# osmarks/meme-search-engine

Hardware: AMD Instinct MI355X
Metric: queries/sec over 1e8x1152 index @ recall@10>=0.95 (exact brute force: recall 1.0) (higher is better)
Workload: dtype f16 in, f32 accumulate, i64 fixed-point scores; 1 GPU; brute-force top-10 over 100000000 x 1152 fp16 rows, 320 queries/step, row-sharded over 1 GPU(s); rows_total=100000000, rows_per_gpu=100000000, k=10, parallelism=row-shard x1

## Files before the change

### meme-search-engine_amd/csrc/scan_mfma.hip

```cpp
#include "common.h"
#include "kernels.h"
#include <cstdlib>
#include <algorithm>
#include <type_traits>

namespace mse {
namespace {

typedef _Float16 half8 __attribute__((ext_vector_type(8)));
typedef float float4v __attribute__((ext_vector_type(4)));
typedef uint32_t u32x4 __attribute__((ext_vector_type(4)));

constexpr int KB = 64;
constexpr int W = 8;
constexpr int TILE_ROWS = 32 * W;

__global__ void pack_queries_kernel(const uint16_t* __restrict__ queries, int d, int bn, int n_rows, uint4* __restrict__ packed) {
    const int nkb = d / KB;
    const int QT_SLOTS = bn * 8;
    const int total = nkb * QT_SLOTS;
    queries += (size_t)blockIdx.y * bn * d;
    n_rows -= blockIdx.y * bn;
    packed += (size_t)blockIdx.y * total;
    for (int idx = blockIdx.x * blockDim.x + threadIdx.x; idx < total; idx += gridDim.x * blockDim.x) {
        const int kb = idx / QT_SLOTS;
        const int r = idx % QT_SLOTS;
        const int q = r >> 3, slot_sw = r & 7;
        const int slot = slot_sw ^ ((q >> 1) & 7);
        packed[idx] = q < n_rows ? *reinterpret_cast<const uint4*>(queries + (size_t)q * d + kb * KB + slot * 8) : uint4{0u, 0u, 0u, 0u};
    }
}

__device__ __forceinline__ half8 as_half8(const u32x4& v) { return __builtin_bit_cast(half8, v); }

template <int N> __device__ __forceinline__ void vm_wait() {
    asm volatile("s_waitcnt vmcnt(%0)" ::"n"(N) : "memory");
    __builtin_amdgcn_sched_barrier(0);
}
__device__ __forceinline__ void dma16(const void* gptr, void* lds_wave_base) {
    __builtin_amdgcn_global_load_lds((const __attribute__((address_space(1))) void*)gptr,
                                     (__attribute__((address_space(3))) void*)lds_wave_base, 16, 0, 0);
}

constexpr float MASKED_OUT = -3.402823466e+38f;
__device__ __forceinline__ uint32_t group_word(size_t group, const uint32_t* words, size_t n_words) {
    return group < n_words ? words[group] : 0u;
}

template <int S, int NCT, int ABL = 0, typename... Mask>
__global__ __launch_bounds__(W * 64) void scan_mfma_kernel(const uint16_t* __restrict__ base, size_t n_rows, int d,
                                                           const uint4* __restrict__ packed_ro,
                                                           float* __restrict__ gmax, int nq_pad, size_t n_tiles, uint32_t y_packed, uint32_t y_cols,
                                                           Mask... mask) {
    constexpr int BN = NCT * 16;
    constexpr int QT_BYTES = BN * 128;
    constexpr int QI = BN / 64;
    constexpr bool ILV = S >= 2 && !(ABL & 16);
    extern __shared__ __attribute__((aligned(16))) char smem[];
    const int tid = threadIdx.x;
    const int lane = tid & 63, wave = tid >> 6;
    const int i = lane & 15, g = lane >> 4;
    const int nkb = d / KB;
    const size_t row_bytes = (size_t)d * 2;
    const int swz = (i >> 1) & 7;
    const size_t n_groups = (n_rows + 31) / 32;
    char* const qbase = smem;
    char* const xbase = smem + 2 * QT_BYTES + wave * (S * 4096);
    gmax += (size_t)blockIdx.y * y_cols;
    const char* const packed = reinterpret_cast<const char*>(packed_ro + (size_t)blockIdx.y * y_packed) + (size_t)(wave * QI * 64 + lane) * 16;

    size_t tile = blockIdx.x;
    if (tile >= n_tiles) return;

    auto src_ptr = [&](size_t t, int u) -> const char* {
        const int r = 8 * u + (lane >> 3);
        size_t row = t * TILE_ROWS + wave * 32 + r;
        if (row >= n_rows) row = n_rows - 1;
        const int piece = (lane & 7) ^ ((r >> 1) & 7);
        return reinterpret_cast<const char*>(base) + row * row_bytes + piece * 16;
    };
    auto dma_x = [&](const char* (&rp)[4], int kblock, int stage) {
        char* dst = xbase + stage * 4096;
        if (ABL & 4) return;
#pragma unroll
        for (int u = 0; u < 4; u++) dma16(rp[u] + (size_t)kblock * 128, dst + u * 1024);
    };
    auto dma_q = [&](int kblock, int qb) {
        const char* src = packed + (size_t)kblock * QT_BYTES;
        char* dst = qbase + qb * QT_BYTES + wave * (QI * 1024);
        if (ABL & 2) return;
#pragma unroll
        for (int u = 0; u < QI; u++) dma16(src + u * 1024, dst + u * 1024);
    };

    const char* rp[4];
    const char* rn[4];
#pragma unroll
    for (int u = 0; u < 4; u++) rp[u] = src_ptr(tile, u);
    dma_q(0, 0);
#pragma unroll
    for (int j = 0; j < S - 1; j++) dma_x(rp, j % nkb, j);
    vm_wait<0>();
    __builtin_amdgcn_s_barrier();

    int buf = 0;
    while (true) {
        float4v acc[2][NCT];
#pragma unroll
        for (int rt = 0; rt < 2; rt++)
#pragma unroll
            for (int ct = 0; ct < NCT; ct++)
#pragma unroll
                for (int r = 0; r < 4; r++) acc[rt][ct][r] = 0.0f;

        const size_t next_tile = tile + gridDim.x;
        const bool has_next_tile = next_tile < n_tiles;
#pragma unroll
        for (int u = 0; u < 4; u++) rn[u] = has_next_tile ? src_ptr(next_tile, u) : rp[u];

        for (int kb0 = 0; kb0 < nkb; kb0 += S) {
#pragma unroll
            for (int j = 0; j < S; j++) {
                const int kb = kb0 + j;
                const int kq = kb + 1 == nkb ? 0 : kb + 1;
                const int kf = kb + S - 1;
                const bool x_next = kf >= nkb;
                const size_t xoff = (size_t)(kf >= nkb ? kf - nkb : kf) * 128;
                char* const xdst = xbase + ((j + S - 1) % S) * 4096;
                const char* const qsrc = packed + (size_t)kq * QT_BYTES;
                char* const qdst = qbase + (buf ^ 1) * QT_BYTES + wave * (QI * 1024);
                auto issue_piece = [&](int p) {
                    if (p < QI) { if (!(ABL & 2)) dma16(qsrc + p * 1024, qdst + p * 1024); }
                    else if (!(ABL & 4)) dma16((x_next ? rn[p - QI] : rp[p - QI]) + xoff, xdst + (p - QI) * 1024);
                };
                if (!ILV) {
#pragma unroll
                    for (int p = 0; p < QI + 4; p++) issue_piece(p);
                    vm_wait<(QI + 4) * (S - 1)>();
                } else if (S == 2) {
                    vm_wait<0>();
                }

                const u32x4* xs = reinterpret_cast<const u32x4*>(xbase + j * 4096) + i * 8;
                const u32x4* qt = reinterpret_cast<const u32x4*>(qbase + buf * QT_BYTES) + i * 8;
                const int slot_a = g ^ swz, slot_b = (4 + g) ^ swz;
                u32x4 bq[2][2];
                bq[0][0] = qt[0 * 128 + slot_a];
                bq[0][1] = qt[1 * 128 + slot_a];
                const half8 a00 = as_half8(xs[slot_a]), a10 = as_half8(xs[128 + slot_a]);
                const half8 a01 = as_half8(xs[slot_b]), a11 = as_half8(xs[128 + slot_b]);
                constexpr int NCP = NCT / 2;
#pragma unroll
                for (int t = 0; t < 2 * NCP; t++) {
                    const int ks = t / NCP, cp = t % NCP;
                    if (t + 1 < 2 * NCP) {
                        const int ks2 = (t + 1) / NCP, cp2 = (t + 1) % NCP;
                        if (!(ABL & 8)) {
                            bq[(t + 1) & 1][0] = qt[(cp2 * 2) * 128 + (ks2 ? slot_b : slot_a)];
                            bq[(t + 1) & 1][1] = qt[(cp2 * 2 + 1) * 128 + (ks2 ? slot_b : slot_a)];
                        } else {
                            bq[(t + 1) & 1][0] = bq[t & 1][1];
                            bq[(t + 1) & 1][1] = bq[t & 1][0];
                        }
                    }
                    __builtin_amdgcn_sched_barrier(0);
                    if (ILV) {
                        constexpr int STEP = (2 * NCP) / (QI + 4);
                        if (t >= 1 && (t - 1) % STEP == 0 && (t - 1) / STEP < QI + 4) {
                            issue_piece((t - 1) / STEP);
                            __builtin_amdgcn_sched_barrier(0);
                        }
                    }
                    const half8 a0 = ks ? a01 : a00;
                    const half8 a1 = ks ? a11 : a10;
#pragma unroll
                    for (int e = 0; e < 2; e++) {
                        const half8 b = as_half8(bq[t & 1][e]);
                        const int ct = cp * 2 + e;
                        if (!(ABL & 1)) {
                            acc[0][ct] = __builtin_amdgcn_mfma_f32_16x16x32_f16(a0, b, acc[0][ct], 0, 0, 0);
                            acc[1][ct] = __builtin_amdgcn_mfma_f32_16x16x32_f16(a1, b, acc[1][ct], 0, 0, 0);
                        } else {
                            asm volatile("" ::"v"(b), "v"(a0), "v"(a1));
                        }
                    }
                }
                vm_wait<4>();
                __builtin_amdgcn_s_barrier();
                buf ^= 1;
            }
        }

        const size_t group = tile * W + wave;
        if constexpr (sizeof...(Mask) != 0) {
            const uint32_t w = group_word(group, mask...) >> (4 * g);
#pragma unroll
            for (int rt = 0; rt < 2; rt++)
#pragma unroll
                for (int r = 0; r < 4; r++) {
                    if ((w >> (16 * rt + r)) & 1u) continue;
#pragma unroll
                    for (int ct = 0; ct < NCT; ct++) acc[rt][ct][r] = MASKED_OUT;
                }
        }
#pragma unroll
        for (int ct = 0; ct < NCT; ct++) {
            float m = fmaxf(fmaxf(acc[0][ct][0], acc[0][ct][1]), fmaxf(acc[0][ct][2], acc[0][ct][3]));
            m = fmaxf(m, fmaxf(fmaxf(acc[1][ct][0], acc[1][ct][1]), fmaxf(acc[1][ct][2], acc[1][ct][3])));
            m = fmaxf(m, __shfl_xor(m, 16));
            m = fmaxf(m, __shfl_xor(m, 32));
            if (g == 0 && group < n_groups) gmax[group * (size_t)nq_pad + ct * 16 + i] = m;
        }

        if (!has_next_tile) break;
        tile = next_tile;
#pragma unroll
        for (int u = 0; u < 4; u++) rp[u] = rn[u];
    }
    vm_wait<0>();
}


typedef float float16v __attribute__((ext_vector_type(16)));

#ifdef MSE_DEV_KERNELS
__device__ unsigned long long g_scan_prof[4];
__device__ __forceinline__ uint32_t memtime() { return (uint32_t)__builtin_amdgcn_s_memtime(); }
#endif

template <typename... M> struct is_tile_subset : std::false_type {};
template <> struct is_tile_subset<ScanSparse> : std::true_type {};
template <typename... M> __device__ __forceinline__ ScanSparse tile_subset_of(const M&...) { return ScanSparse{}; }
__device__ __forceinline__ ScanSparse tile_subset_of(const ScanSparse& sp) { return sp; }

template <int S, int MF, int PROF = 0, int BN = 256, int GR = 32, typename... Mask>
__global__ __launch_bounds__(W * 64) void scan_mfma2d_kernel(const uint16_t* __restrict__ base, size_t n_rows, int d,
                                                             const uint4* __restrict__ packed_ro,
                                                             float* __restrict__ gmax, int nq_pad, size_t n_tiles, uint32_t y_packed, uint32_t y_cols,
                                                             Mask... mask) {
    constexpr bool SPF = is_tile_subset<Mask...>::value;
    constexpr bool MASKED = sizeof...(Mask) != 0 && !SPF;
    static_assert(sizeof...(Mask) == 0 || (MF == 16 && PROF == 0), "the masked form is the product kernel's");
    static_assert(!SPF || (BN == 320 && GR == 64), "a tile subset: the 320-query search pass only");
    static_assert(BN == 256 || (BN == 320 && MF == 16 && S == 2), "320 queries: 16x16x32 tiles on the two-stage ring only");
    static_assert(GR == 32 || (GR == 64 && MF == 16), "rows per written maximum: 32, or the wave's 64");
    constexpr int HALF = BN / 2;
    constexpr int QT_BYTES = BN * 128;
    constexpr int QI = BN / 64;
    constexpr bool XF = S == 2 && PROF != 4;
    constexpr int CLOSE = S == 2 ? 0 : 4;
    constexpr int RG_BYTES = 64 * 128;
    extern __shared__ __attribute__((aligned(16))) char smem[];
    const int tid = threadIdx.x;
    const int lane = tid & 63, wave = is_tile_subset<Mask...>::value ? __builtin_amdgcn_readfirstlane(tid >> 6) : tid >> 6;
    const int rg = wave >> 1, qh = wave & 1;
    const int nkb = d / KB;
    const size_t row_bytes = (size_t)d * 2;
    const size_t n_groups = (n_rows + GR - 1) / GR;
    char* const qbase = smem;
    char* const xbase = smem + 2 * QT_BYTES + rg * (S * RG_BYTES);
    gmax += (size_t)blockIdx.y * y_cols;
    const char* const packed = reinterpret_cast<const char*>(packed_ro + (size_t)blockIdx.y * y_packed) + (size_t)(wave * QI * 64 + lane) * 16;

    const ScanSparse sp = tile_subset_of(mask...);
    const size_t n_vt = SPF ? sp.n_tiles : n_tiles;
    auto tile_of = [&](size_t v) -> size_t { return SPF ? v * sp.mul + (v >> sp.shift) + sp.add : v; };
    size_t vt = blockIdx.x;
    if (vt >= n_vt) return;
    size_t tile = tile_of(vt);

    auto src_ptr = [&](size_t t, int u) -> const char* {
        const int r = qh * 32 + 8 * u + (lane >> 3);
        size_t row = t * TILE_ROWS + rg * 64 + r;
        if (row >= n_rows) row = n_rows - 1;
        const int piece = (lane & 7) ^ ((r >> 1) & 7);
        return reinterpret_cast<const char*>(base) + row * row_bytes + piece * 16;
    };
    const char* rp[4];
    const char* rn[4];
#pragma unroll
    for (int u = 0; u < 4; u++) rp[u] = src_ptr(tile, u);
    {
        char* qdst = qbase + wave * (QI * 1024);
#pragma unroll
        for (int u = 0; u < QI; u++) dma16(packed + u * 1024, qdst + u * 1024);
#pragma unroll
        for (int j = 0; j < S - 1; j++)
#pragma unroll
            for (int u = 0; u < 4; u++) dma16(rp[u] + (size_t)(j % nkb) * 128, xbase + j * RG_BYTES + (qh * 4 + u) * 1024);
    }
    vm_wait<0>();
    __builtin_amdgcn_s_barrier();

    const int i = MF == 16 ? (lane & 15) : (lane & 31);
    const int g = MF == 16 ? (lane >> 4) : (lane >> 5);
    const int swz = (i >> 1) & 7;
    constexpr int NKS = MF == 16 ? 2 : 4;
    constexpr int NRT = 64 / MF, NCTW = HALF / MF;
    constexpr int NACC = MF == 16 ? 4 : 16;
    typedef typename std::conditional<MF == 16, float4v, float16v>::type accv;

    int buf = 0;
#ifdef MSE_DEV_KERNELS
    uint32_t pt_issue = 0, pt_wait = 0, pt_bar = 0, pt_n = 0, pt_last = 0;
    if constexpr (PROF == 1) pt_last = memtime();
#endif
    while (true) {
        accv acc[NRT][NCTW];
#pragma unroll
        for (int rt = 0; rt < NRT; rt++)
#pragma unroll
            for (int ct = 0; ct < NCTW; ct++)
#pragma unroll
                for (int r = 0; r < NACC; r++) acc[rt][ct][r] = 0.0f;

        const size_t next_vt = vt + gridDim.x;
        const size_t next_tile = tile_of(next_vt);
        const bool has_next_tile = next_vt < n_vt;
#pragma unroll
        for (int u = 0; u < 4; u++) rn[u] = has_next_tile ? src_ptr(next_tile, u) : rp[u];

        for (int kb0 = 0; kb0 < nkb; kb0 += S) {
#pragma unroll
            for (int j = 0; j < S; j++) {
                const int kb = kb0 + j;
                const int kq = kb + 1 == nkb ? 0 : kb + 1;
                const int kf = kb + S - 1;
                const bool x_next = kf >= nkb;
                const size_t xoff = (size_t)(kf >= nkb ? kf - nkb : kf) * 128;
                char* const xdst = xbase + ((j + S - 1) % S) * RG_BYTES + qh * 4096;
                const char* const qsrc = packed + (size_t)kq * QT_BYTES;
                char* const qdst = qbase + (buf ^ 1) * QT_BYTES + wave * (QI * 1024);
                auto issue_piece = [&](int p) {
                    const int pq = XF ? p - 4 : p, px = XF ? p : p - QI;
                    if (XF ? p >= 4 : p < QI) dma16(qsrc + pq * 1024, qdst + pq * 1024);
                    else dma16((x_next ? rn[px] : rp[px]) + xoff, xdst + px * 1024);
                };

                const u32x4* xs = reinterpret_cast<const u32x4*>(xbase + j * RG_BYTES) + i * 8;
                const u32x4* qt = reinterpret_cast<const u32x4*>(qbase + buf * QT_BYTES) + (qh * HALF + i) * 8;
                auto slot = [&](int ks) { return (MF == 16 ? (4 * ks + g) : (2 * ks + g)) ^ swz; };
                half8 a[2][NRT];
#pragma unroll
                for (int rt = 0; rt < NRT; rt++) a[0][rt] = as_half8(xs[rt * (MF * 8) + slot(0)]);
                constexpr int NT = NKS * NCTW;
                u32x4 bq[3];
                bq[0] = qt[0 * (MF * 8) + slot(0)];
                bq[1] = qt[1 * (MF * 8) + slot(0)];
#pragma unroll
                for (int t = 0; t < NT; t++) {
                    const int ks = t / NCTW, ct = t % NCTW;
                    if (t + 2 < NT) bq[(t + 2) % 3] = qt[((t + 2) % NCTW) * (MF * 8) + slot((t + 2) / NCTW)];
                    if (ct == NCTW - 2 && ks + 1 < NKS) {
#pragma unroll
                        for (int rt = 0; rt < NRT; rt++) a[(ks + 1) & 1][rt] = as_half8(xs[rt * (MF * 8) + slot(ks + 1)]);
                    }
                    __builtin_amdgcn_sched_barrier(0);
                    {
                        constexpr int STEP = NT / (QI + 4);
                        int pc = -1;
                        if constexpr (S == 2 && PROF != 4 && PROF != 5 && !MASKED) {
                            if (t >= 1 && t <= 4) pc = t - 1;
                            else if (t >= 6 && (t - 6) % 2 == 0 && (t - 6) / 2 < QI) pc = 4 + (t - 6) / 2;
                        } else if (t >= 1 && (t - 1) % STEP == 0 && (t - 1) / STEP < QI + 4) pc = (t - 1) / STEP;
                        if (pc >= 0) {
                            issue_piece(pc);
                            __builtin_amdgcn_sched_barrier(0);
                        }
                    }
                    const half8 b = as_half8(bq[t % 3]);
                    if constexpr (PROF == 3) __builtin_amdgcn_s_setprio(1);
#pragma unroll
                    for (int rt = 0; rt < NRT; rt++) {
                        if constexpr (MF == 16) acc[rt][ct] = __builtin_amdgcn_mfma_f32_16x16x32_f16(a[ks & 1][rt], b, acc[rt][ct], 0, 0, 0);
                        else acc[rt][ct] = __builtin_amdgcn_mfma_f32_32x32x16_f16(a[ks & 1][rt], b, acc[rt][ct], 0, 0, 0);
                    }
                    if constexpr (PROF == 3) __builtin_amdgcn_s_setprio(0);
                }
#ifdef MSE_DEV_KERNELS
                if constexpr (PROF == 1) {
                    const uint32_t t0 = memtime();
                    vm_wait<CLOSE>();
                    const uint32_t t1 = memtime();
                    __builtin_amdgcn_s_barrier();
                    const uint32_t t2 = memtime();
                    pt_issue += t0 - pt_last; pt_wait += t1 - t0; pt_bar += t2 - t1; pt_n++; pt_last = t2;
                } else
#endif
                {
                    vm_wait<CLOSE>();
#ifdef MSE_DEV_KERNELS
                    if constexpr (PROF != 2)
#endif
                    __builtin_amdgcn_s_barrier();
                }
                buf ^= 1;
            }
        }

        if constexpr (MASKED && GR == 32) {
#pragma unroll
            for (int p = 0; p < 2; p++) {
                const uint32_t w = group_word(tile * W + rg * 2 + p, mask...) >> (4 * g);
#pragma unroll
                for (int h = 0; h < 2; h++)
#pragma unroll
                    for (int r = 0; r < 4; r++) {
                        if ((w >> (16 * h + r)) & 1u) continue;
#pragma unroll
                        for (int ct = 0; ct < NCTW; ct++) acc[2 * p + h][ct][r] = MASKED_OUT;
                    }
            }
        }
        if constexpr (GR == 64) {
            const size_t group = tile * 4 + rg;
            uint32_t allowed = 0xFFFFu;
            if constexpr (MASKED) {
                const uint32_t w0 = group_word(group * 2, mask...) >> (4 * g), w1 = group_word(group * 2 + 1, mask...) >> (4 * g);
                allowed = (w0 & 15u) | ((w0 >> 16 & 15u) << 4) | ((w1 & 15u) << 8) | ((w1 >> 16 & 15u) << 12);
            }
            auto av = [&](int rt, int ct, int r) {
                if constexpr (MASKED) return (allowed >> (4 * rt + r)) & 1u ? acc[rt][ct][r] : MASKED_OUT;
                else return acc[rt][ct][r];
            };
            float tq[3] = {0.0f, 0.0f, 0.0f};
            uint32_t cbase = (uint32_t)(qh * HALF + i);
            if constexpr (SPF) {
                asm volatile("" : "+v"(cbase));
                if (sp.tau) {
#pragma unroll
                    for (int j = 0; j < 3; j++) tq[j] = g + 4 * j < NCTW ? sp.tau[cbase + (g + 4 * j) * MF] : __builtin_inff();
                }
            }
#pragma unroll
            for (int ct = 0; ct < NCTW; ct++) {
                float m = fmaxf(fmaxf(av(0, ct, 0), av(0, ct, 1)), fmaxf(av(0, ct, 2), av(0, ct, 3)));
#pragma unroll
                for (int rt = 1; rt < 4; rt++)
                    m = fmaxf(m, fmaxf(fmaxf(av(rt, ct, 0), av(rt, ct, 1)), fmaxf(av(rt, ct, 2), av(rt, ct, 3))));
                m = fmaxf(m, __shfl_xor(m, 16));
                m = fmaxf(m, __shfl_xor(m, 32));
#ifdef MSE_DEV_KERNELS
                if constexpr (PROF == 6) { asm volatile("" ::"v"(m)); continue; }
#endif
                if constexpr (SPF) {
                    if (sp.tau) {
                        const uint32_t col = cbase + ct * MF;
                        if (g == (ct & 3) && group < n_groups && m > tq[ct >> 2]) {
                            uint32_t one;
                            asm volatile("v_mov_b32 %0, 1" : "=v"(one));
                            const uint32_t pos = atomicAdd(&sp.counts[col], one);
                            if (pos < sp.cap) {
                                sp.ids[col * sp.cap + pos] = (uint32_t)group;
                                sp.keys[col * sp.cap + pos] = m;
                            }
                        }
                    } else if (g == 0 && group < n_groups) {
                        gmax[(vt * 4 + rg) * (size_t)nq_pad + cbase + ct * MF] = m;
                    }
                    __builtin_amdgcn_sched_barrier(0);
                    continue;
                }
                if (g == 0 && group < n_groups) gmax[group * (size_t)nq_pad + qh * HALF + ct * MF + i] = m;
            }
        } else {
#pragma unroll
            for (int p = 0; p < 2; p++) {
                const size_t group = tile * W + rg * 2 + p;
#pragma unroll
                for (int ct = 0; ct < NCTW; ct++) {
                    float m;
                    if constexpr (MF == 16) {
                        m = fmaxf(fmaxf(acc[2 * p][ct][0], acc[2 * p][ct][1]), fmaxf(acc[2 * p][ct][2], acc[2 * p][ct][3]));
                        m = fmaxf(m, fmaxf(fmaxf(acc[2 * p + 1][ct][0], acc[2 * p + 1][ct][1]), fmaxf(acc[2 * p + 1][ct][2], acc[2 * p + 1][ct][3])));
                        m = fmaxf(m, __shfl_xor(m, 16));
                        m = fmaxf(m, __shfl_xor(m, 32));
                    } else {
                        m = acc[p][ct][0];
#pragma unroll
                        for (int r = 1; r < 16; r++) m = fmaxf(m, acc[p][ct][r]);
                        m = fmaxf(m, __shfl_xor(m, 32));
                    }
                    if (g == 0 && group < n_groups) gmax[group * (size_t)nq_pad + qh * HALF + ct * MF + i] = m;
                }
            }
        }

        if (!has_next_tile) break;
        vt = next_vt;
        tile = next_tile;
#pragma unroll
        for (int u = 0; u < 4; u++) rp[u] = rn[u];
#ifdef MSE_DEV_KERNELS
        if constexpr (PROF == 1) pt_last = memtime();
#endif
    }
    vm_wait<0>();
#ifdef MSE_DEV_KERNELS
    if constexpr (PROF == 1) {
        if (lane == 0) {
            atomicAdd(&g_scan_prof[0], (unsigned long long)pt_issue); atomicAdd(&g_scan_prof[1], (unsigned long long)pt_wait);
            atomicAdd(&g_scan_prof[2], (unsigned long long)pt_bar); atomicAdd(&g_scan_prof[3], (unsigned long long)pt_n);
        }
    }
#endif
}


#ifdef MSE_DEV_KERNELS

template <int S>
__global__ __launch_bounds__(W * 64) void scan_mfma2s_kernel(const uint16_t* __restrict__ base, size_t n_rows, int d,
                                                             const uint4* __restrict__ packed_ro,
                                                             float* __restrict__ gmax, int nq_pad, size_t n_tiles, uint32_t y_packed, uint32_t y_cols) {
    static_assert(S == 3, "the specialised schedule is written for the 3-stage ring");
    constexpr int BN = 256;
    constexpr int QT_BYTES = BN * 128;
    constexpr int RG_BYTES = 64 * 128;
    constexpr int NP = 8;
    extern __shared__ __attribute__((aligned(16))) char smem[];
    const int tid = threadIdx.x;
    const int lane = tid & 63;
    const int wave = __builtin_amdgcn_readfirstlane(tid >> 6);
    const int rg = wave >> 1, qh = wave & 1;
    const bool row_wave = wave < 4;
    const int w4 = wave & 3;
    const int nkb = d / KB;
    const size_t row_bytes = (size_t)d * 2;
    char* const qbase = smem;
    char* const xring = smem + 2 * QT_BYTES;
    char* const xbase = xring + rg * (S * RG_BYTES);
    char* const xfill = xring + w4 * (S * RG_BYTES);
    char* const qfill = qbase + w4 * (NP * 1024);
    gmax += (size_t)blockIdx.y * y_cols;
    const char* const packed = reinterpret_cast<const char*>(packed_ro + (size_t)blockIdx.y * y_packed) + (size_t)w4 * (NP * 1024) + lane * 16;

    size_t tile = blockIdx.x;
    if (tile >= n_tiles) return;

    const size_t lane_off = (size_t)(lane >> 3) * row_bytes + (size_t)(((lane & 7) ^ (lane >> 4)) * 16);
    const char* const rows0 = reinterpret_cast<const char*>(base) + (size_t)w4 * 64 * row_bytes;
    auto tile_ptr = [&](size_t t) { return rows0 + t * TILE_ROWS * row_bytes + lane_off; };
    const char* lp = tile_ptr(tile);
    const char* ln = lp;
    const size_t piece_rows = 8 * row_bytes;
    auto dma_row_piece = [&](const char* p, int u, size_t koff, char* dst) {
        const char* q = (u & 1) ? reinterpret_cast<const char*>(reinterpret_cast<uintptr_t>(p) ^ 64u) : p;
        dma16(q + (u * piece_rows + koff), dst + u * 1024);
    };
    if (row_wave) {
#pragma unroll
        for (int j = 0; j < S - 1; j++)
#pragma unroll
            for (int u = 0; u < NP; u++) dma_row_piece(lp, u, (size_t)(j % nkb) * 128, xfill + j * RG_BYTES);
    } else {
#pragma unroll
        for (int u = 0; u < NP; u++) dma16(packed + u * 1024, qfill + u * 1024);
    }
    vm_wait<0>();
    __builtin_amdgcn_s_barrier();

    const int i = lane & 15, g = lane >> 4;
    const int swz = (i >> 1) & 7;
    int buf = 0;
    while (true) {
        float4v acc[4][8];
#pragma unroll
        for (int rt = 0; rt < 4; rt++)
#pragma unroll
            for (int ct = 0; ct < 8; ct++)
#pragma unroll
                for (int r = 0; r < 4; r++) acc[rt][ct][r] = 0.0f;

        const size_t next_tile = tile + gridDim.x;
        const bool has_next_tile = next_tile < n_tiles;
        ln = has_next_tile ? tile_ptr(next_tile) : lp;

        for (int kb0 = 0; kb0 < nkb; kb0 += S) {
#pragma unroll
            for (int j = 0; j < S; j++) {
                const int kb = kb0 + j;
                const int kq = kb + 1 == nkb ? 0 : kb + 1;
                const int kf = kb + S - 1;
                const char* const xp = kf >= nkb ? ln : lp;
                const size_t xoff = (size_t)(kf >= nkb ? kf - nkb : kf) * 128;
                char* const xdst = xfill + ((j + S - 1) % S) * RG_BYTES;
                const char* const qsrc = packed + (size_t)kq * QT_BYTES;
                char* const qdst = qfill + (buf ^ 1) * QT_BYTES;
                auto issue_piece = [&](int p) {
                    if (row_wave) dma_row_piece(xp, p, xoff, xdst);
                    else dma16(qsrc + p * 1024, qdst + p * 1024);
                };

                const u32x4* xs = reinterpret_cast<const u32x4*>(xbase + j * RG_BYTES) + i * 8;
                const u32x4* qt = reinterpret_cast<const u32x4*>(qbase + buf * QT_BYTES) + (qh * 128 + i) * 8;
                auto slot = [&](int ks) { return (4 * ks + g) ^ swz; };
                half8 a[2][4];
#pragma unroll
                for (int rt = 0; rt < 4; rt++) a[0][rt] = as_half8(xs[rt * 128 + slot(0)]);
                u32x4 bq[3];
                bq[0] = qt[0 * 128 + slot(0)];
                bq[1] = qt[1 * 128 + slot(0)];
#pragma unroll
                for (int t = 0; t < 16; t++) {
                    const int ks = t / 8, ct = t % 8;
                    if (t + 2 < 16) bq[(t + 2) % 3] = qt[((t + 2) % 8) * 128 + slot((t + 2) / 8)];
                    if (ct == 6 && ks == 0) {
#pragma unroll
                        for (int rt = 0; rt < 4; rt++) a[1][rt] = as_half8(xs[rt * 128 + slot(1)]);
                    }
                    __builtin_amdgcn_sched_barrier(0);
                    if (t >= 1 && (t - 1) % 2 == 0 && (t - 1) / 2 < NP) {
                        issue_piece((t - 1) / 2);
                        __builtin_amdgcn_sched_barrier(0);
                    }
                    const half8 b = as_half8(bq[t % 3]);
#pragma unroll
                    for (int rt = 0; rt < 4; rt++) acc[rt][ct] = __builtin_amdgcn_mfma_f32_16x16x32_f16(a[ks][rt], b, acc[rt][ct], 0, 0, 0);
                }
                if (row_wave) vm_wait<NP>(); else vm_wait<0>();
                __builtin_amdgcn_s_barrier();
                buf ^= 1;
            }
        }

#pragma unroll
        for (int p = 0; p < 2; p++) {
            const size_t group = tile * W + rg * 2 + p;
#pragma unroll
            for (int ct = 0; ct < 8; ct++) {
                float m = fmaxf(fmaxf(acc[2 * p][ct][0], acc[2 * p][ct][1]), fmaxf(acc[2 * p][ct][2], acc[2 * p][ct][3]));
                m = fmaxf(m, fmaxf(fmaxf(acc[2 * p + 1][ct][0], acc[2 * p + 1][ct][1]), fmaxf(acc[2 * p + 1][ct][2], acc[2 * p + 1][ct][3])));
                m = fmaxf(m, __shfl_xor(m, 16));
                m = fmaxf(m, __shfl_xor(m, 32));
                if (g == 0) gmax[group * (size_t)nq_pad + qh * 128 + ct * 16 + i] = m;
            }
        }
        if (!has_next_tile) break;
        tile = next_tile;
        lp = ln;
    }
    vm_wait<0>();
}
#endif

thread_local unsigned g_pass_count = 1;
thread_local uint32_t g_pass_packed = 0, g_pass_cols = 0;

template <typename K, typename... Mask>
int launch_kernel(K kernel, size_t lds, size_t grid, hipStream_t stream, const uint16_t* base, size_t n_rows, int d,
                  const uint4* packed, float* group_max, int nq_pad, Mask... mask) {
    const size_t n_tiles = (n_rows + TILE_ROWS - 1) / TILE_ROWS;
    if (grid > n_tiles) grid = n_tiles;
    MSE_DYN_LDS(kernel, lds);
    hipLaunchKernelGGL(kernel, dim3((unsigned)grid, g_pass_count), dim3(W * 64), lds, stream, base, n_rows, d, packed, group_max, nq_pad, n_tiles,
                       g_pass_packed, g_pass_cols, mask...);
    MSE_HIP_TRY(hipGetLastError());
    return 0;
}

template <int S, int NCT, int ABL, typename... Mask>
int launch_variant(size_t grid, hipStream_t stream, const uint16_t* base, size_t n_rows, int d, const uint4* packed,
                   float* group_max, int nq_pad, Mask... mask) {
    const size_t lds = 2 * (size_t)(NCT * 16 * 128) + (size_t)W * S * 4096;
    return launch_kernel(scan_mfma_kernel<S, NCT, ABL, Mask...>, lds, grid, stream, base, n_rows, d, packed, group_max, nq_pad, mask...);
}

#ifdef MSE_DEV_KERNELS

template <int S>
int launch_2s(size_t grid, hipStream_t stream, const uint16_t* base, size_t n_rows, int d, const uint4* packed,
              float* group_max, int nq_pad) {
    const size_t lds = 2 * (size_t)(256 * 128) + (size_t)4 * S * 8192;
    const size_t n_full = n_rows / TILE_ROWS * TILE_ROWS;
    if (n_full && launch_kernel(scan_mfma2s_kernel<S>, lds, grid, stream, base, n_full, d, packed, group_max, nq_pad)) return -1;
    if (n_full < n_rows)
        return launch_variant<S, 16, 0>(1, stream, base + n_full * (size_t)d, n_rows - n_full, d, packed,
                                        group_max + (n_full / 32) * (size_t)nq_pad, nq_pad);
    return 0;
}
#endif

template <int S, int MF, int PROF = 0, int BN = 256, int GR = 32, typename... Mask>
int launch_2d(size_t grid, hipStream_t stream, const uint16_t* base, size_t n_rows, int d, const uint4* packed,
              float* group_max, int nq_pad, Mask... mask) {
    const size_t lds = 2 * (size_t)(BN * 128) + (size_t)4 * S * 8192;
    return launch_kernel(scan_mfma2d_kernel<S, MF, PROF, BN, GR, Mask...>, lds, grid, stream, base, n_rows, d, packed, group_max, nq_pad, mask...);
}

}

int mfma_query_tile(int d) { return (d / KB) % 2 == 0 ? 320 : 256; }
int mfma_pad(int nq, int d) {
    if (nq <= 128) return 128;
    if (nq <= 192 && (d / KB) % 3 == 0) return 192;
    if (nq <= 256 || (d / KB) % 2 != 0) return 256;
    return 320;
}

size_t mfma_packed_bytes(int d) { return (size_t)(d / KB) * 320 * 128; }

#ifndef MSE_GROUP_ROWS_320
#define MSE_GROUP_ROWS_320 64
#endif
int mfma_group_rows(int nq_pad) {
#ifdef MSE_DEV_KERNELS
    if (getenv("MSE_SCAN_2D") || (getenv("MSE_SCAN_ABL") && atoi(getenv("MSE_SCAN_ABL")) != 32)) return 32;
#endif
    return nq_pad == 320 ? MSE_GROUP_ROWS_320 : 32;
}

int launch_scan_mfma(const uint16_t* base, size_t n_rows, int d, const uint16_t* queries_dev, int nq_pad,
                     void* packed_scratch, float* group_max, int n_cu, hipStream_t stream, hipEvent_t ev_begin,
                     hipEvent_t ev_end, int gm_stride, int n_pass, const uint32_t* mask, size_t mask_words, int nq_rows, int group_rows) {
    if (n_rows == 0) return 0;
    if (group_rows != 32 && !(group_rows == 64 && nq_pad == 320)) return fail("scan_mfma: 32 rows per group maximum, or 64 on the 320-query pass");
    if (nq_rows < 0) nq_rows = n_pass * nq_pad;
    if (n_pass < 1 || n_pass > 65535) return fail("scan_mfma: 1..65535 passes per launch");
    if (n_pass > 1 && !gm_stride) return fail("scan_mfma: batched passes need a common group-maximum stride");
    const int gs = gm_stride ? gm_stride : nq_pad;
    if (gs < nq_pad) return fail("scan_mfma: group-maximum stride below the pass width");
    if (d % 64 != 0 || d <= 0 || d > D_MAX) return fail("vector width must be a positive multiple of 64");
    if (nq_pad != 128 && nq_pad != 256 && !(nq_pad == 192 && (d / KB) % 3 == 0) && !(nq_pad == 320 && (d / KB) % 2 == 0))
        return fail("scan_mfma: query tile must be padded to 128, 192 (K blocks divisible by 3), 256 or 320 (K blocks even)");
    uint4* packed = reinterpret_cast<uint4*>(packed_scratch);
    hipLaunchKernelGGL(pack_queries_kernel, dim3(64, (unsigned)n_pass), dim3(256), 0, stream, queries_dev, d, nq_pad, nq_rows, packed);
    struct PassScope {
        PassScope(unsigned n, uint32_t pk, uint32_t cols) { g_pass_count = n; g_pass_packed = pk; g_pass_cols = cols; }
        ~PassScope() { g_pass_count = 1; g_pass_packed = 0; g_pass_cols = 0; }
    } pass_scope((unsigned)n_pass, (uint32_t)((size_t)(d / KB) * nq_pad * 8), (uint32_t)nq_pad);
    if (ev_begin) MSE_HIP_TRY(hipEventRecord(ev_begin, stream));
    const int nkb = d / KB;
    const int S = nkb % 3 == 0 ? 3 : nkb % 2 == 0 ? 2 : 1;
    const size_t grid = (size_t)n_cu;
    int rc = -2;
#ifdef MSE_DEV_KERNELS
    if (!mask && group_rows == 32) {
    const int abl = getenv("MSE_SCAN_ABL") ? atoi(getenv("MSE_SCAN_ABL")) : 0;
    const int v2d = getenv("MSE_SCAN_2D") ? atoi(getenv("MSE_SCAN_2D")) : -1;
    if (nq_pad == 128 && S == 3 && abl == 16) rc = launch_variant<3, 8, 16>(grid, stream, base, n_rows, d, packed, group_max, gs);
    else if (nq_pad == 256 && S == 3 && abl) {
        switch (abl) {
            case 1: rc = launch_variant<3, 16, 1>(grid, stream, base, n_rows, d, packed, group_max, gs); break;
            case 2: rc = launch_variant<3, 16, 2>(grid, stream, base, n_rows, d, packed, group_max, gs); break;
            case 4: rc = launch_variant<3, 16, 4>(grid, stream, base, n_rows, d, packed, group_max, gs); break;
            case 6: rc = launch_variant<3, 16, 6>(grid, stream, base, n_rows, d, packed, group_max, gs); break;
            case 8: rc = launch_variant<3, 16, 8>(grid, stream, base, n_rows, d, packed, group_max, gs); break;
            case 9: rc = launch_variant<3, 16, 9>(grid, stream, base, n_rows, d, packed, group_max, gs); break;
            case 14: rc = launch_variant<3, 16, 14>(grid, stream, base, n_rows, d, packed, group_max, gs); break;
            case 16: rc = launch_variant<3, 16, 16>(grid, stream, base, n_rows, d, packed, group_max, gs); break;
            default: break;
        }
    }
    else if (nq_pad == 320 && v2d == 0) rc = launch_variant<2, 20, 0>(grid, stream, base, n_rows, d, packed, group_max, gs);
    else if (nq_pad == 320 && v2d == 165) rc = launch_2d<2, 16, 5, 320>(grid, stream, base, n_rows, d, packed, group_max, gs);
    else if (nq_pad == 320 && v2d == 164) rc = launch_2d<2, 16, 4, 320>(grid, stream, base, n_rows, d, packed, group_max, gs);
    else if (nq_pad == 256 && S == 3 && v2d == 0) rc = launch_variant<3, 16, 0>(grid, stream, base, n_rows, d, packed, group_max, gs);
    else if (nq_pad == 256 && S == 3 && v2d == 161) rc = launch_2d<3, 16, 1>(grid, stream, base, n_rows, d, packed, group_max, gs);
    else if (nq_pad == 256 && S == 3 && v2d == 162) rc = launch_2d<3, 16, 2>(grid, stream, base, n_rows, d, packed, group_max, gs);
    else if (nq_pad == 256 && S == 3 && v2d == 163) rc = launch_2d<3, 16, 3>(grid, stream, base, n_rows, d, packed, group_max, gs);
    else if (nq_pad == 256 && S == 3 && v2d == 17) rc = launch_2s<3>(grid, stream, base, n_rows, d, packed, group_max, gs);
    else if (nq_pad == 256 && S == 3 && v2d == 32) rc = launch_2d<3, 32>(grid, stream, base, n_rows, d, packed, group_max, gs);
    }
    if (!mask && group_rows == 64 && nq_pad == 320 && getenv("MSE_SCAN_ABL") && atoi(getenv("MSE_SCAN_ABL")) == 32)
        rc = launch_2d<2, 16, 6, 320, 64>(grid, stream, base, n_rows, d, packed, group_max, gs);
    if (rc != -2) {
        if (rc) return rc;
        if (ev_end) MSE_HIP_TRY(hipEventRecord(ev_end, stream));
        return 0;
    }
#endif
    auto run = [&](auto launch) { return mask ? launch(mask, mask_words) : launch(); };
    if (nq_pad == 320) {
        if (group_rows == 64) rc = run([&](auto... m) { return launch_2d<2, 16, 0, 320, 64>(grid, stream, base, n_rows, d, packed, group_max, gs, m...); });
        else rc = run([&](auto... m) { return launch_2d<2, 16, 0, 320>(grid, stream, base, n_rows, d, packed, group_max, gs, m...); });
    } else if (nq_pad == 192) {
        rc = run([&](auto... m) { return launch_variant<3, 12, 0>(grid, stream, base, n_rows, d, packed, group_max, gs, m...); });
    } else if (nq_pad == 128) {
        if (S == 3) rc = run([&](auto... m) { return launch_variant<3, 8, 0>(grid, stream, base, n_rows, d, packed, group_max, gs, m...); });
        else if (S == 2) rc = run([&](auto... m) { return launch_variant<2, 8, 0>(grid, stream, base, n_rows, d, packed, group_max, gs, m...); });
        else rc = run([&](auto... m) { return launch_variant<1, 8, 0>(grid, stream, base, n_rows, d, packed, group_max, gs, m...); });
    } else {
        if (S == 3) rc = run([&](auto... m) { return launch_2d<3, 16>(grid, stream, base, n_rows, d, packed, group_max, gs, m...); });
        else if (S == 2) rc = run([&](auto... m) { return launch_variant<2, 16, 0>(grid, stream, base, n_rows, d, packed, group_max, gs, m...); });
        else rc = run([&](auto... m) { return launch_variant<1, 16, 0>(grid, stream, base, n_rows, d, packed, group_max, gs, m...); });
    }
    if (rc) return rc;
    if (ev_end) MSE_HIP_TRY(hipEventRecord(ev_end, stream));
    return 0;
}

int launch_scan_mfma_tiles(const uint16_t* base, size_t n_rows, int d, const uint16_t* queries_dev, int nq_rows, bool pack, void* packed_scratch,
                           const ScanSparse& sp, float* group_max, int n_cu, hipStream_t stream, hipEvent_t ev_begin, hipEvent_t ev_end) {
    if (n_rows == 0) return 0;
    if (d % 64 != 0 || d <= 0 || d > D_MAX || (d / KB) % 2 != 0) return fail("scan_mfma_tiles: the 320-query pass needs an even number of K blocks");
    if (sp.tau ? !(sp.counts && sp.ids && sp.keys && sp.cap) : !group_max) return fail("scan_mfma_tiles: no place for the maxima");
    constexpr int BN = 320;
    uint4* packed = reinterpret_cast<uint4*>(packed_scratch);
    if (pack) hipLaunchKernelGGL(pack_queries_kernel, dim3(64, 1), dim3(256), 0, stream, queries_dev, d, BN, nq_rows, packed);
    if (ev_begin) MSE_HIP_TRY(hipEventRecord(ev_begin, stream));
    if (sp.n_tiles) {
        auto kernel = scan_mfma2d_kernel<2, 16, 0, BN, 64, ScanSparse>;
        const size_t lds = 2 * (size_t)(BN * 128) + (size_t)4 * 2 * 8192;
        const size_t n_tiles = (n_rows + TILE_ROWS - 1) / TILE_ROWS;
        const size_t grid = std::min<size_t>((size_t)n_cu, sp.n_tiles);
        MSE_DYN_LDS(kernel, lds);
        hipLaunchKernelGGL(kernel, dim3((unsigned)grid, 1), dim3(W * 64), lds, stream, base, n_rows, d, (const uint4*)packed, group_max, BN, n_tiles,
                           0u, 0u, sp);
        MSE_HIP_TRY(hipGetLastError());
    }
    if (ev_end) MSE_HIP_TRY(hipEventRecord(ev_end, stream));
    return 0;
}

}

#ifdef MSE_DEV_KERNELS
extern "C" __attribute__((visibility("default"))) int mse_dev_scan_prof(unsigned long long out[4]) {
    unsigned long long z[4] = {0, 0, 0, 0};
    if (hipMemcpyFromSymbol(out, HIP_SYMBOL(mse::g_scan_prof), sizeof(z)) != hipSuccess) return -1;
    if (hipMemcpyToSymbol(HIP_SYMBOL(mse::g_scan_prof), z, sizeof(z)) != hipSuccess) return -1;
    return 0;
}
#endif
```

Measured before the change: 4768 queries/s.

## Transpose group-max reduction with permlane swaps, stage tau in LDS, cheapen tile turnover

```diff
diff --git a/meme-search-engine_amd/csrc/scan_mfma.hip b/meme-search-engine_amd/csrc/scan_mfma.hip
--- a/meme-search-engine_amd/csrc/scan_mfma.hip
+++ b/meme-search-engine_amd/csrc/scan_mfma.hip
@@ -14,6 +14,7 @@
 constexpr int KB = 64;
 constexpr int W = 8;
 constexpr int TILE_ROWS = 32 * W;
+constexpr int TAU_SLOTS = 384;
 
 __global__ void pack_queries_kernel(const uint16_t* __restrict__ queries, int d, int bn, int n_rows, uint4* __restrict__ packed) {
     const int nkb = d / KB;
@@ -224,7 +225,7 @@
 typedef float float16v __attribute__((ext_vector_type(16)));
 
 #ifdef MSE_DEV_KERNELS
-__device__ unsigned long long g_scan_prof[4];
+__device__ unsigned long long g_scan_prof[6];
 __device__ __forceinline__ uint32_t memtime() { return (uint32_t)__builtin_amdgcn_s_memtime(); }
 #endif
 
@@ -240,7 +241,8 @@
                                                              Mask... mask) {
     constexpr bool SPF = is_tile_subset<Mask...>::value;
     constexpr bool MASKED = sizeof...(Mask) != 0 && !SPF;
-    static_assert(sizeof...(Mask) == 0 || (MF == 16 && PROF == 0), "the masked form is the product kernel's");
+    static_assert(sizeof...(Mask) == 0 || (MF == 16 && (PROF == 0 || (PROF == 1 && is_tile_subset<Mask...>::value))),
+                  "the masked form is the product kernel's");
     static_assert(!SPF || (BN == 320 && GR == 64), "a tile subset: the 320-query search pass only");
     static_assert(BN == 256 || (BN == 320 && MF == 16 && S == 2), "320 queries: 16x16x32 tiles on the two-stage ring only");
     static_assert(GR == 32 || (GR == 64 && MF == 16), "rows per written maximum: 32, or the wave's 64");
@@ -250,9 +252,10 @@
     constexpr bool XF = S == 2 && PROF != 4;
     constexpr int CLOSE = S == 2 ? 0 : 4;
     constexpr int RG_BYTES = 64 * 128;
+    constexpr bool TURN = BN == 320 && GR == 64;
     extern __shared__ __attribute__((aligned(16))) char smem[];
     const int tid = threadIdx.x;
-    const int lane = tid & 63, wave = is_tile_subset<Mask...>::value ? __builtin_amdgcn_readfirstlane(tid >> 6) : tid >> 6;
+    const int lane = tid & 63, wave = TURN ? __builtin_amdgcn_readfirstlane(tid >> 6) : tid >> 6;
     const int rg = wave >> 1, qh = wave & 1;
     const int nkb = d / KB;
     const size_t row_bytes = (size_t)d * 2;
@@ -289,6 +292,11 @@
 #pragma unroll
             for (int u = 0; u < 4; u++) dma16(rp[u] + (size_t)(j % nkb) * 128, xbase + j * RG_BYTES + (qh * 4 + u) * 1024);
     }
+    float* const tau_lds = reinterpret_cast<float*>(smem + 2 * QT_BYTES + 4 * S * RG_BYTES);
+    if constexpr (SPF) {
+        if (sp.tau && tid < TAU_SLOTS) tau_lds[tid] = tid < BN ? sp.tau[tid] : __builtin_inff();
+        __builtin_amdgcn_fence(__ATOMIC_RELEASE, "workgroup");
+    }
     vm_wait<0>();
     __builtin_amdgcn_s_barrier();
 
@@ -302,7 +310,7 @@
 
     int buf = 0;
 #ifdef MSE_DEV_KERNELS
-    uint32_t pt_issue = 0, pt_wait = 0, pt_bar = 0, pt_n = 0, pt_last = 0;
+    uint32_t pt_issue = 0, pt_wait = 0, pt_bar = 0, pt_n = 0, pt_last = 0, pt_turn = 0, pt_tiles = 0;
     if constexpr (PROF == 1) pt_last = memtime();
 #endif
     while (true) {
@@ -317,10 +325,28 @@
         const size_t next_vt = vt + gridDim.x;
         const size_t next_tile = tile_of(next_vt);
         const bool has_next_tile = next_vt < n_vt;
-#pragma unroll
-        for (int u = 0; u < 4; u++) rn[u] = has_next_tile ? src_ptr(next_tile, u) : rp[u];
-
-        for (int kb0 = 0; kb0 < nkb; kb0 += S) {
+        if (TURN && has_next_tile && (tile + 1) * TILE_ROWS <= n_rows && (next_tile + 1) * TILE_ROWS <= n_rows) {
+            const size_t ahead = (next_tile - tile) * TILE_ROWS * row_bytes;
+#pragma unroll
+            for (int u = 0; u < 4; u++) rn[u] = rp[u] + ahead;
+        } else {
+#pragma unroll
+            for (int u = 0; u < 4; u++) rn[u] = has_next_tile ? src_ptr(next_tile, u) : rp[u];
+        }
+
+#ifdef MSE_DEV_KERNELS
+        if constexpr (PROF == 1) {
+#pragma unroll
+            for (int rt = 0; rt < NRT; rt++)
+#pragma unroll
+                for (int ct = 0; ct < NCTW; ct++) asm volatile("" : "+v"(acc[rt][ct]));
+            __builtin_amdgcn_sched_barrier(0);
+            const uint32_t t = memtime();
+            pt_turn += t - pt_last; pt_last = t;
+            __builtin_amdgcn_sched_barrier(0);
+        }
+#endif
+        for (int kb0 = 0; kb0 < nkb || (TURN && kb0 == 0); kb0 += S) {
 #pragma unroll
             for (int j = 0; j < S; j++) {
                 const int kb = kb0 + j;
@@ -423,45 +449,59 @@
                 if constexpr (MASKED) return (allowed >> (4 * rt + r)) & 1u ? acc[rt][ct][r] : MASKED_OUT;
                 else return acc[rt][ct][r];
             };
-            float tq[3] = {0.0f, 0.0f, 0.0f};
+            static_assert(NCTW == 10, "the transposed reduction below is laid out for the ten column tiles of the 320-query kernel");
             uint32_t cbase = (uint32_t)(qh * HALF + i);
-            if constexpr (SPF) {
-                asm volatile("" : "+v"(cbase));
-                if (sp.tau) {
-#pragma unroll
-                    for (int j = 0; j < 3; j++) tq[j] = g + 4 * j < NCTW ? sp.tau[cbase + (g + 4 * j) * MF] : __builtin_inff();
+            asm volatile("" : "+v"(cbase));
+            float m[NCTW];
+#pragma unroll
+            for (int ct = 0; ct < NCTW; ct++) {
+                float x = av(0, ct, 0);
+#pragma unroll
+                for (int e = 1; e + 1 < 16; e += 2) x = fmaxf(fmaxf(x, av(e >> 2, ct, e & 3)), av((e + 1) >> 2, ct, (e + 1) & 3));
+                m[ct] = fmaxf(x, av(3, ct, 3));
+            }
+            auto swap_max = [](float a, float b, auto half) {
+                uint32_t ua = __builtin_bit_cast(uint32_t, a), ub = __builtin_bit_cast(uint32_t, b);
+                uint32_t r0, r1;
+                if constexpr (decltype(half)::value) {
+                    const auto r = __builtin_amdgcn_permlane32_swap(ua, ub, false, false);
+                    r0 = r[0]; r1 = r[1];
+                } else {
+                    const auto r = __builtin_amdgcn_permlane16_swap(ua, ub, false, false);
+                    r0 = r[0]; r1 = r[1];
                 }
-            }
-#pragma unroll
-            for (int ct = 0; ct < NCTW; ct++) {
-                float m = fmaxf(fmaxf(av(0, ct, 0), av(0, ct, 1)), fmaxf(av(0, ct, 2), av(0, ct, 3)));
-#pragma unroll
-                for (int rt = 1; rt < 4; rt++)
-                    m = fmaxf(m, fmaxf(fmaxf(av(rt, ct, 0), av(rt, ct, 1)), fmaxf(av(rt, ct, 2), av(rt, ct, 3))));
-                m = fmaxf(m, __shfl_xor(m, 16));
-                m = fmaxf(m, __shfl_xor(m, 32));
-#ifdef MSE_DEV_KERNELS
-                if constexpr (PROF == 6) { asm volatile("" ::"v"(m)); continue; }
+                return fmaxf(__builtin_bit_cast(float, r0), __builtin_bit_cast(float, r1));
+            };
+            float p[5], q[3];
+#pragma unroll
+            for (int j = 0; j < 5; j++) p[j] = swap_max(m[2 * j], m[2 * j + 1], std::false_type{});
+            q[0] = swap_max(p[0], p[1], std::true_type{});
+            q[1] = swap_max(p[2], p[3], std::true_type{});
+            q[2] = swap_max(p[4], p[4], std::true_type{});
+#pragma unroll
+            for (int j = 0; j < 3; j++) {
+                const uint32_t col = cbase + (4 * j + g) * MF;
+                const bool mine = (j < 2 || g < 2) && group < n_groups;
+#ifdef MSE_DEV_KERNELS
+                if constexpr (PROF == 6) { asm volatile("" ::"v"(q[j])); continue; }
 #endif
                 if constexpr (SPF) {
                     if (sp.tau) {
-                        const uint32_t col = cbase + ct * MF;
-                        if (g == (ct & 3) && group < n_groups && m > tq[ct >> 2]) {
+                        if (mine && q[j] > tau_lds[col]) {
                             uint32_t one;
                             asm volatile("v_mov_b32 %0, 1" : "=v"(one));
                             const uint32_t pos = atomicAdd(&sp.counts[col], one);
                             if (pos < sp.cap) {
                                 sp.ids[col * sp.cap + pos] = (uint32_t)group;
-                                sp.keys[col * sp.cap + pos] = m;
+                                sp.keys[col * sp.cap + pos] = q[j];
                             }
                         }
-                    } else if (g == 0 && group < n_groups) {
-                        gmax[(vt * 4 + rg) * (size_t)nq_pad + cbase + ct * MF] = m;
-                    }
-                    __builtin_amdgcn_sched_barrier(0);
-                    continue;
+                    } else if (mine) {
+                        gmax[(vt * 4 + rg) * (size_t)nq_pad + col] = q[j];
+                    }
+                } else if (mine) {
+                    gmax[group * (size_t)nq_pad + col] = q[j];
                 }
-                if (g == 0 && group < n_groups) gmax[group * (size_t)nq_pad + qh * HALF + ct * MF + i] = m;
             }
         } else {
 #pragma unroll
@@ -486,14 +526,19 @@
             }
         }
 
+#ifdef MSE_DEV_KERNELS
+        if constexpr (PROF == 1) {
+            __builtin_amdgcn_sched_barrier(0);
+            const uint32_t t = memtime();
+            pt_turn += t - pt_last; pt_last = t; pt_tiles++;
+            __builtin_amdgcn_sched_barrier(0);
+        }
+#endif
         if (!has_next_tile) break;
         vt = next_vt;
         tile = next_tile;
 #pragma unroll
         for (int u = 0; u < 4; u++) rp[u] = rn[u];
-#ifdef MSE_DEV_KERNELS
-        if constexpr (PROF == 1) pt_last = memtime();
-#endif
     }
     vm_wait<0>();
 #ifdef MSE_DEV_KERNELS
@@ -501,6 +546,7 @@
         if (lane == 0) {
             atomicAdd(&g_scan_prof[0], (unsigned long long)pt_issue); atomicAdd(&g_scan_prof[1], (unsigned long long)pt_wait);
             atomicAdd(&g_scan_prof[2], (unsigned long long)pt_bar); atomicAdd(&g_scan_prof[3], (unsigned long long)pt_n);
+            atomicAdd(&g_scan_prof[4], (unsigned long long)pt_turn); atomicAdd(&g_scan_prof[5], (unsigned long long)pt_tiles);
         }
     }
 #endif
@@ -705,7 +751,7 @@
 #endif
 int mfma_group_rows(int nq_pad) {
 #ifdef MSE_DEV_KERNELS
-    if (getenv("MSE_SCAN_2D") || (getenv("MSE_SCAN_ABL") && atoi(getenv("MSE_SCAN_ABL")) != 32)) return 32;
+    if (getenv("MSE_SCAN_2D") || (getenv("MSE_SCAN_ABL") && atoi(getenv("MSE_SCAN_ABL")) != 32 && atoi(getenv("MSE_SCAN_ABL")) != 33)) return 32;
 #endif
     return nq_pad == 320 ? MSE_GROUP_ROWS_320 : 32;
 }
@@ -764,6 +810,8 @@
     }
     if (!mask && group_rows == 64 && nq_pad == 320 && getenv("MSE_SCAN_ABL") && atoi(getenv("MSE_SCAN_ABL")) == 32)
         rc = launch_2d<2, 16, 6, 320, 64>(grid, stream, base, n_rows, d, packed, group_max, gs);
+    if (!mask && group_rows == 64 && nq_pad == 320 && getenv("MSE_SCAN_ABL") && atoi(getenv("MSE_SCAN_ABL")) == 33)
+        rc = launch_2d<2, 16, 1, 320, 64>(grid, stream, base, n_rows, d, packed, group_max, gs);
     if (rc != -2) {
         if (rc) return rc;
         if (ev_end) MSE_HIP_TRY(hipEventRecord(ev_end, stream));
@@ -801,7 +849,10 @@
     if (ev_begin) MSE_HIP_TRY(hipEventRecord(ev_begin, stream));
     if (sp.n_tiles) {
         auto kernel = scan_mfma2d_kernel<2, 16, 0, BN, 64, ScanSparse>;
-        const size_t lds = 2 * (size_t)(BN * 128) + (size_t)4 * 2 * 8192;
+#ifdef MSE_DEV_KERNELS
+        if (getenv("MSE_SCAN_ABL") && atoi(getenv("MSE_SCAN_ABL")) == 33) kernel = scan_mfma2d_kernel<2, 16, 1, BN, 64, ScanSparse>;
+#endif
+        const size_t lds = 2 * (size_t)(BN * 128) + (size_t)4 * 2 * 8192 + TAU_SLOTS * sizeof(float);
         const size_t n_tiles = (n_rows + TILE_ROWS - 1) / TILE_ROWS;
         const size_t grid = std::min<size_t>((size_t)n_cu, sp.n_tiles);
         MSE_DYN_LDS(kernel, lds);
@@ -816,8 +867,8 @@
 }
 
 #ifdef MSE_DEV_KERNELS
-extern "C" __attribute__((visibility("default"))) int mse_dev_scan_prof(unsigned long long out[4]) {
-    unsigned long long z[4] = {0, 0, 0, 0};
+extern "C" __attribute__((visibility("default"))) int mse_dev_scan_prof(unsigned long long out[6]) {
+    unsigned long long z[6] = {0, 0, 0, 0, 0, 0};
     if (hipMemcpyFromSymbol(out, HIP_SYMBOL(mse::g_scan_prof), sizeof(z)) != hipSuccess) return -1;
     if (hipMemcpyToSymbol(HIP_SYMBOL(mse::g_scan_prof), z, sizeof(z)) != hipSuccess) return -1;
     return 0;
```

Result: faster. 4887 queries/s, median of 6 (+2.5%).
